# near/near-light-client

Measured on AMD Instinct MI355X. Metric: Sync/Verify proofs/sec at 1/2/4/8 MI355X + achieved HBM GB/s vs roofline, higher is better.
Workload: dtype u64 (Goldilocks field, integer)

## Files before the change

### near-light-client_amd/airgen.py

```python
import os
import sys
import types

import numpy as np

HERE = os.path.dirname(os.path.abspath(__file__))
OUT_DIR = os.path.join(HERE, "csrc", "airgen")
P = 0xFFFFFFFF00000001
MASK64 = (1 << 64) - 1

(LOCAL, NEXT, PUBLIC, CONST, ADD, SUB, MUL, EMIT_TRANSITION, EMIT_FIRST, EMIT_LAST, EMIT, PERIODIC, PACK_LOCAL, PACK_NEXT, EMIT_BOOL,
 LOADV, XOR3, CH, MAJ, SEGMENT, EMIT_LOGUP, MAC) = range(22)


def program_hash(words):
    h = 0xcbf29ce484222325
    for b in np.ascontiguousarray(words, dtype="<u8").tobytes():
        h = ((h ^ b) * 0x100000001b3) & MASK64
    return h


def canonical_words(words):
    out, i = [int(w) for w in words], 0
    while i < len(out):
        if (out[i] & 0xFF) == CONST:
            out[i + 1] %= P
            i += 2
        else:
            i += 1
    return np.array(out, dtype=np.uint64)


def _segments(words):
    segs, lo, i = [], 0, 0
    while i < len(words):
        op = int(words[i]) & 0xFF
        if op == SEGMENT:
            segs.append((lo, i))
            lo = i + 1
        i += 2 if op == CONST else 1
    segs.append((lo, len(words)))
    return segs


HORNER = "acc0 = gl::add_loose(gl::mul_loose(acc0, g.a0), %s); acc1 = gl::add_loose(gl::mul_loose(acc1, g.a1), %s);"
HORNER_SEGMENTS = {
    "ed25519_2p7_tagged": (2646, 6297, 6956, 7679, 8370, 9093, 14490, 15181, 15872),
    "sha512_tagged": (8982, 10259, 11536, 12813, 14090, 15367, 16644, 17921, 19198, 20475, 21752, 23029, 24306, 25583, 26144, 26705,
                      27266),
}


def segment_exponents(words, lo, hi):
    n, i = 0, lo
    while i < hi:
        w = int(words[i])
        op = w & 0xFF
        if op in (EMIT_TRANSITION, EMIT_FIRST, EMIT_LAST, EMIT):
            n += 1
        elif op == EMIT_LOGUP:
            n += 2
        elif op == EMIT_BOOL:
            n += ((w >> 40) & 0xFFFF) or 1
        i += 2 if op == CONST else 1
    return [n - 1 - k for k in range(n)]


class _Fold:

    def __init__(self, exponents, wide):
        self.exponents, self.wide, self.k = exponents, wide, 0

    def emit(self, lines, expr, indent="    ", canonical=False):
        if self.wide:
            e = self.exponents[self.k]
            lines.append("%sacc.mac(%s, AP0(%d), AP1(%d));" % (indent, expr if canonical else expr.replace("gl::mul(", "gl::mul_loose(", 1), e, e))
        else:
            lines.append("%sc = %s; " % (indent, expr) + HORNER % ("c", "c"))
        self.k += 1


SCHED_EVERY = 4


def _segment_body(words, lo, hi, wide=False):
    L, i, since = [], lo, 0
    fold = _Fold(segment_exponents(words, lo, hi), wide)
    R = lambda k: "r%d" % k
    while i < hi:
        if since >= SCHED_EVERY:
            L.append("    __builtin_amdgcn_sched_barrier(0);")
            since = 0
        if (int(words[i]) & 0xFF) in (LOCAL, NEXT, PUBLIC, CONST, ADD, SUB, MUL, PERIODIC, PACK_LOCAL, PACK_NEXT, XOR3, CH, MAJ, MAC):
            since += 1
        w = int(words[i])
        op, dst, a, b, sh = w & 0xFF, (w >> 8) & 0xFFFF, (w >> 24) & 0xFFFF, (w >> 40) & 0xFFFF, (w >> 56) & 0x3F
        i += 1
        if op == LOCAL:
            L.append("    %s = COL(%d, g.row);" % (R(dst), a))
        elif op == NEXT:
            L.append("    %s = COL(%d, g.row_next);" % (R(dst), a))
        elif op == PUBLIC:
            L.append("    %s = PIS(%d);" % (R(dst), a))
        elif op == PERIODIC:
            L.append("    %s = g.per[(size_t)%d * g.per_stride + g.per_off];" % (R(dst), a))
        elif op == CONST:
            L.append("    %s = 0x%016xull;" % (R(dst), int(words[i]) % P))
            i += 1
        elif op == ADD:
            L.append("    %s = gl::add(%s, mul_pow2(%s, %d));" % (R(dst), R(a), R(b), sh) if sh else "    %s = gl::add(%s, %s);" % (R(dst), R(a), R(b)))
        elif op == SUB:
            L.append("    %s = gl::sub(%s, mul_pow2(%s, %d));" % (R(dst), R(a), R(b), sh) if sh else "    %s = gl::sub(%s, %s);" % (R(dst), R(a), R(b)))
        elif op == MUL:
            L.append("    %s = gl::mul(%s, %s);" % (R(dst), R(a), R(b)))
        elif op == MAC:
            L.append("    %s = gl::add(%s, gl::mul(%s, %s));" % (R(dst), R(sh), R(a), R(b)))
        elif op == CH:
            L.append("    %s = gl::add(%s, gl::mul(%s, gl::sub(%s, %s)));" % (R(dst), R(sh), R(a), R(b), R(sh)))
        elif op in (XOR3, MAJ):
            L.append("    { const uint64_t xy = gl::mul(%s, %s), sx = gl::sub(gl::add(%s, %s), gl::add(xy, xy));" % (R(a), R(b), R(a), R(b)))
            if op == XOR3:
                L.append("      const uint64_t sz = gl::mul(sx, %s); %s = gl::sub(gl::add(sx, %s), gl::add(sz, sz)); }" % (R(sh), R(dst), R(sh)))
            else:
                L.append("      %s = gl::add(xy, gl::mul(%s, sx)); }" % (R(dst), R(sh)))
        elif op in (PACK_LOCAL, PACK_NEXT):
            row = "g.row" if op == PACK_LOCAL else "g.row_next"
            L.append("    { uint64_t v[%d];" % b)
            for k in range(b):
                L.append("      v[%d] = COL(%d, %s);" % (k, a + k, row))
            L.append("      uint64_t acc = 0;")
            for k in range(b):
                L.append("      acc = gl::add(acc, mul_pow2(v[%d], %d));" % (k, k))
            L.append("      %s = acc; }" % R(dst))
        elif op == EMIT_BOOL:
            cnt = b if b else 1
            for i0 in range(0, cnt, 8):
                m = min(8, cnt - i0)
                L.append("    { uint64_t v[%d];" % m)
                for k in range(m):
                    L.append("      v[%d] = COL(%d, g.row);" % (k, a + i0 + k))
                for k in range(m):
                    fold.emit(L, "gl::mul(v[%d], gl::sub(v[%d], 1))" % (k, k), indent="      ")
                L.append("    }")
        elif op == EMIT_LOGUP:
            L.append("    { const uint64_t al0 = PIS(g.n_pis + %d), al1 = PIS(g.n_pis + %d);" % (sh, sh + 1))
            L.append("      const uint64_t h0 = COL(%d, g.row), h1 = COL(%d, g.row), v1 = COL(%d, g.row);" % (b, b + 1, a))
            L.append("      uint64_t c0, c1;")
            if dst == 0xFFFF:
                L.append("      const uint64_t d0 = gl::add(al0, v1);")
                L.append("      c0 = gl::sub(gl::add(gl::mul(h0, d0), mul_pow2(gl::mul(h1, al1), 3)), gl::add(gl::mul(h1, al1), 1));")
                L.append("      c1 = gl::add(gl::mul(h0, al1), gl::mul(h1, d0));")
            else:
                L.append("      const uint64_t v2 = COL(%d, g.row);" % dst)
                L.append("      const uint64_t s2 = gl::add(gl::add(al0, al0), gl::add(v1, v2));")
                L.append("      const uint64_t a1sq = gl::mul(al1, al1);")
                L.append("      const uint64_t u0 = gl::add(gl::mul(gl::add(al0, v1), gl::add(al0, v2)), gl::sub(mul_pow2(a1sq, 3), a1sq));")
                L.append("      const uint64_t u1 = gl::mul(al1, s2);")
                L.append("      const uint64_t hu = gl::mul(h1, u1);")
                L.append("      c0 = gl::sub(gl::add(gl::mul(h0, u0), gl::sub(mul_pow2(hu, 3), hu)), s2);")
                L.append("      c1 = gl::sub(gl::add(gl::mul(h0, u1), gl::mul(h1, u0)), gl::add(al1, al1));")
            fold.emit(L, "c0", indent="      ", canonical=True)
            fold.emit(L, "c1", indent="      ", canonical=True)
            L.append("    }")
        elif op == LOADV:
            L.append("    __builtin_amdgcn_sched_barrier(0);")
        elif op == EMIT_TRANSITION:
            fold.emit(L, "gl::mul(%s, g.z_last)" % R(a))
        elif op == EMIT_FIRST:
            fold.emit(L, "gl::mul(%s, g.l_first)" % R(a))
        elif op == EMIT_LAST:
            fold.emit(L, "gl::mul(%s, g.l_last)" % R(a))
        elif op == EMIT:
            fold.emit(L, R(a), canonical=True)
        else:
            raise ValueError("unknown opcode %d at word %d" % (op, i - 1))
    assert fold.k == len(fold.exponents)
    return L


def _registers_of(words, lo, hi):
    regs, i = set(), lo
    while i < hi:
        w = int(words[i])
        op = w & 0xFF
        if op in (LOCAL, NEXT, PUBLIC, CONST, ADD, SUB, MUL, PERIODIC, PACK_LOCAL, PACK_NEXT, XOR3, CH, MAJ, MAC):
            regs.add((w >> 8) & 0xFFFF)
        i += 2 if op == CONST else 1
    return sorted(regs)


PART_WORDS = 10000


def generate_sources(name, words):
    words = canonical_words(words)
    h = program_hash(words)
    segs = _segments(words)
    parts, cur, cur_words = [], [], 0
    for lo, hi in segs:
        if cur and cur_words + (hi - lo) > PART_WORDS:
            parts.append(cur)
            cur, cur_words = [], 0
        cur.append((lo, hi))
        cur_words += hi - lo
    parts.append(cur)
    files = {}
    for pi, part in enumerate(parts):
        ns = "airgen_%s_p%d" % (name, pi)
        out = ["// GENERATED by near-light-client_amd/airgen.py from the program words of AIR '%s' (%d words, %d segments, hash 0x%016x):" % (name, len(words), len(segs), h),
               "// part %d of %d, segments starting at words %s." % (pi + 1, len(parts), ", ".join(str(lo) for lo, _ in part)),
               "// Do not edit: the interpreter k_air_quotient (stark.hip) runs the same words and is the parity reference.",
               '#include "../air_vm.hpp"', "", "namespace nlx {", "namespace %s {" % ns, "",
               "// what a segment needs of the point: passed BY VALUE (registers); the wave-uniform members are made scalar again inside",
               "// the function (readfirstlane), so a column's base address is a scalar load and its element ONE vector load",
               "// The column-pointer table and the public inputs are the same for every lane and constant for the launch: read through the",
               "// constant address space they are scalar loads (s_load), and a column's value is then ONE global load with the pointer in",
               "// SGPRs and the row's byte offset in a VGPR.  Through plain pointers hipcc made each a per-lane flat load with a wait",
               "// between the pointer and the value (two memory latencies per column, two more VGPRs per load in flight).",
               "// row / row_next are BYTE offsets (LDE rows * 8 < 2^32: the host selects these kernels for LDEs of <= 2^28 rows only).",
               "typedef const uint64_t __attribute__((address_space(4)))* airgen_kptr;",
               "typedef const char __attribute__((address_space(1)))* airgen_gptr;",
               "#define COL(c, off) (*(const uint64_t __attribute__((address_space(1)))*)((airgen_gptr)((airgen_kptr)g.cols)[c] + (off)))",
               "#define PIS(i) (((airgen_kptr)g.pis)[i])",
               "#define AP0(j) (((airgen_kptr)g.ap0)[j])",
               "#define AP1(j) (((airgen_kptr)g.ap1)[j])",
               "struct G {", "    uint64_t cols, pis, ap0, ap1; const uint64_t* per;",
               "    size_t per_stride, per_off; uint64_t a0, a1, z_last, l_first, l_last; uint32_t row, row_next, n_pis;", "};",
               "struct Acc { uint64_t a0, a1; };",
               "template <typename T> __device__ __forceinline__ T* uni(T* p) {",
               "    const uint64_t v = (uint64_t)p;",
               "    return (T*)(((uint64_t)(uint32_t)__builtin_amdgcn_readfirstlane((int)(v >> 32)) << 32) | (uint32_t)__builtin_amdgcn_readfirstlane((int)v));",
               "}",
               "__device__ __forceinline__ uint64_t uni(uint64_t v) {",
               "    return ((uint64_t)(uint32_t)__builtin_amdgcn_readfirstlane((int)(v >> 32)) << 32) | (uint32_t)__builtin_amdgcn_readfirstlane((int)v);",
               "}", ""]
        for lo, hi in part:
            regs = _registers_of(words, lo, hi)
            out.append("static __device__ __noinline__ Acc seg_%d(G gv) {" % lo)
            out.append("    G g = gv;")
            out.append("    g.cols = uni(gv.cols); g.pis = uni(gv.pis); g.per = uni(gv.per); g.per_stride = uni((uint64_t)gv.per_stride);")
            out.append("    g.a0 = uni(gv.a0); g.a1 = uni(gv.a1); g.n_pis = (uint32_t)__builtin_amdgcn_readfirstlane((int)gv.n_pis);")
            wide = lo not in HORNER_SEGMENTS.get(name, ())
            if wide:
                out.append("    g.ap0 = uni(gv.ap0); g.ap1 = uni(gv.ap1);")
                out.append("    GateAcc acc;")
                out.append("    acc.reset();")
            else:
                out.append("    uint64_t c, acc0 = 0, acc1 = 0;")
            if regs:
                out.append("    uint64_t %s;" % ", ".join("r%d" % r for r in regs))
            out += _segment_body(words, lo, hi, wide)
            if wide:
                out.append("    return Acc{GateAcc::fold_columns(acc.a, acc.kc), GateAcc::fold_columns(acc.a + 4, acc.kc + 4)};")
            else:
                out.append("    return Acc{acc0, acc1};")
            out.append("}")
            out.append("")
        out += [
            "// the interpreter's prologue and epilogue (csrc/stark.hip k_air_quotient), the program between them as a switch on the segment",
            "__global__ __launch_bounds__(AIRGEN_BLOCK) void kernel(AirParams p) {",
            "    const uint32_t sg = blockIdx.y;",
            "    const uint32_t first = p.n_seg > 1 ? p.seg[2 * sg] : 0u;",
            "    if (%s) return;   // another part's segment" % " && ".join("first != %du" % lo for lo, _ in part),
            "    const size_t pos = (size_t)blockIdx.x * blockDim.x + threadIdx.x;",
            "    const unsigned log_Q = p.log_n + p.qdb;",
            "    if (pos >> log_Q) return;",
            "    const size_t n = (size_t)1 << p.log_n;",
            "    const uint32_t rq = (uint32_t)(pos >> p.log_n), k = (uint32_t)(pos & (n - 1));",
            "    const uint32_t r = rq << (p.rate_bits - p.qdb);",
            "    const size_t qrow_next = ((size_t)rq << p.log_n) + ((k + 1) & (n - 1));",
            "    const uint64_t x = gl::mul(p.coset_base[rq], root_pow_(p.w_n_table, k, (uint32_t)(n >> 1)));",
            "    const uint64_t zh = gl::inv(p.zh_inv[rq]);",
            "    G g;",
            "    g.cols = (uint64_t)p.cols; g.pis = (uint64_t)p.pis; g.per = p.periodic; g.n_pis = p.n_pis;",
            "    g.row = (uint32_t)((((size_t)r << p.log_n) + k) << 3); g.row_next = (uint32_t)((((size_t)r << p.log_n) + ((k + 1) & (n - 1))) << 3);",
            "    g.per_stride = (size_t)1 << (p.qdb + p.period_bits);",
            "    g.per_off = ((size_t)rq << p.period_bits) + (k & ((1u << p.period_bits) - 1));",
            "    g.a0 = p.alphas[0]; g.a1 = p.alphas[1];",
            "    g.ap0 = (uint64_t)p.alpha_pows; g.ap1 = (uint64_t)(p.alpha_pows + p.alpha_stride);",
            "    g.z_last = gl::sub(x, p.g_inv); g.l_first = gl::mul(zh, p.l_inv[pos]); g.l_last = gl::mul(zh, p.l_inv[qrow_next]);",
            "    Acc acc{0, 0};",
            "    switch (first) {",
        ]
        for lo, _ in part:
            out.append("        case %d: acc = seg_%d(g); break;" % (lo, lo))
        out += [
            "        default: break;",
            "    }",
            "    const size_t Q = (size_t)1 << log_Q;",
            "    if (p.n_seg > 1) {",
            "        uint64_t* dst = p.part + (((size_t)sg * p.nc) << log_Q) + pos;",
            "        dst[0] = gl::mul(acc.a0, p.seg_mul[2 * sg]);",
            "        dst[Q] = gl::mul(acc.a1, p.seg_mul[2 * sg + 1]);",
            "        return;",
            "    }",
            "    const uint64_t zi = p.zh_inv[rq];",
            "    p.out[pos] = gl::mul(acc.a0, zi);",
            "    p.out[Q + pos] = gl::mul(acc.a1, zi);",
            "}",
            "",
            "}  // namespace %s" % ns,
            "void airgen_launch_%s_p%d(hipStream_t st, unsigned tiles, unsigned n_segments, const AirParams& p) {" % (name, pi),
            "    hipLaunchKernelGGL(%s::kernel, dim3(tiles, n_segments), dim3(AIRGEN_BLOCK), 0, st, p);" % ns,
            "}",
            "}  // namespace nlx", ""]
        files["air_%s_p%d.hip" % (name, pi)] = "\n".join(out)
    main = ["// GENERATED by near-light-client_amd/airgen.py: AIR '%s' (%d words, %d segments in %d parts, hash 0x%016x)." % (name, len(words), len(segs), len(parts), h),
            '#include "../air_vm.hpp"', "", "namespace nlx {"]
    main += ["void airgen_launch_%s_p%d(hipStream_t st, unsigned tiles, unsigned n_segments, const AirParams& p);" % (name, pi) for pi in range(len(parts))]
    main += ["static void airgen_launch_%s(hipStream_t st, unsigned tiles, unsigned n_segments, const AirParams& p) {" % name]
    main += ["    airgen_launch_%s_p%d(st, tiles, n_segments, p);" % (name, pi) for pi in range(len(parts))]
    main += ["}",
             "#if !defined(__HIP_DEVICE_COMPILE__)   // a host object (it holds a host function's address): not for the device pass",
             'extern const AirGenEntry airgen_entry_%s = {0x%016xull, %du, "%s", airgen_launch_%s};' % (name, h, len(words), name, name),
             "#endif",
             "}  // namespace nlx", ""]
    files["air_%s.hip" % name] = "\n".join(main)
    return files


def registry_source(names):
    out = ["// GENERATED by near-light-client_amd/airgen.py: the table nlx_stark_build searches (csrc/air_vm.hpp airgen_find).",
           '#include "../air_vm.hpp"', "", "namespace nlx {"]
    out += ["extern const AirGenEntry airgen_entry_%s;" % n for n in names]
    out += ["", "#if !defined(__HIP_DEVICE_COMPILE__)", "const AirGenEntry* airgen_find(uint64_t program_hash, uint32_t n_words) {",
            "    static const AirGenEntry* const table[] = {%s};" % ", ".join(["&airgen_entry_%s" % n for n in names] + ["nullptr"]),
            "    for (const AirGenEntry* const* e = table; *e; e++)",
            "        if ((*e)->program_hash == program_hash && (*e)->n_words == n_words) return *e;",
            "    return nullptr;", "}", "#endif", "}  // namespace nlx", ""]
    return "\n".join(out)


def _load_air_modules():
    if "nlx_amd" in sys.modules and hasattr(sys.modules["nlx_amd"], "stark"):
        return sys.modules["nlx_amd"]
    import importlib
    pkg = types.ModuleType("nlx_amd")
    pkg.__path__ = [HERE]
    sys.modules["nlx_amd"] = pkg
    lib = types.ModuleType("nlx_amd._lib")

    class NlxError(RuntimeError):
        pass
    lib.dll, lib.synth_dll, lib.ptr, lib.NlxError = None, None, (lambda a: None), NlxError
    sys.modules["nlx_amd._lib"] = lib
    for m in ("stark", "logup", "fp25519", "sha256_air", "sha512_air", "ed25519_air"):
        setattr(pkg, m, importlib.import_module("nlx_amd." + m))
    return pkg


def fixed_programs():
    pkg = _load_air_modules()
    progs = [("sha256_tagged", pkg.sha256_air.sha256_air(tagged=True).compile()),
             ("sha256", pkg.sha256_air.sha256_air(tagged=False).compile()),
             ("sha512_tagged", pkg.sha512_air.sha512_air(tagged=True).compile()),
             ("ed25519_2p7_tagged", pkg.ed25519_air.Ed25519Stark(7, tagged=True).stark.program)]
    return progs


def sources():
    progs = fixed_programs()
    files = {}
    for name, words in progs:
        files.update(generate_sources(name, words))
    files["registry.hip"] = registry_source([name for name, _ in progs])
    return files


def write_all(out_dir=OUT_DIR):
    os.makedirs(out_dir, exist_ok=True)
    files = sources()
    for stale in os.listdir(out_dir):
        if stale.endswith(".hip") and stale not in files:
            os.remove(os.path.join(out_dir, stale))
    for fn, text in files.items():
        path = os.path.join(out_dir, fn)
        if not os.path.exists(path) or open(path).read() != text:
            with open(path, "w") as f:
                f.write(text)
    return sorted(files)


if __name__ == "__main__":
    for fn in write_all():
        print(os.path.join(OUT_DIR, fn))
```

### near-light-client_amd/csrc/gl.hpp

```cpp
#pragma once
#include <stdint.h>
#include <stddef.h>
#include "nlx_field.h"

#if defined(__HIP__)
#include <hip/hip_runtime.h>
#define GL_HD __host__ __device__ __forceinline__
#define GL_H __host__ inline
#else
#define GL_HD inline
#define GL_H inline
#endif

namespace gl {

constexpr uint64_t P = 0xFFFFFFFF00000001ULL;
constexpr uint64_t EPS = 0xFFFFFFFFULL;
constexpr uint64_t GEN = NLX_GL_MULTIPLICATIVE_GROUP_GENERATOR;
constexpr uint64_t POW2_GEN = NLX_GL_POWER_OF_TWO_GENERATOR;
constexpr unsigned TWO_ADICITY = 32;
constexpr uint64_t W = 7;

GL_HD uint64_t mulhi64(uint64_t a, uint64_t b) {
#if defined(__HIP_DEVICE_COMPILE__)
    return __umul64hi(a, b);
#else
    return (uint64_t)(((unsigned __int128)a * b) >> 64);
#endif
}

#if defined(__HIP__)
__device__ __forceinline__ uint64_t canon(uint64_t a) {
    uint64_t t, c;
    asm("v_mad_u64_u32 %[t], %[c], -1, 1, %[a]" : [t] "=&v"(t), [c] "=s"(c) : [a] "v"(a));
    uint32_t r0, r1;
    asm("v_cndmask_b32_e64 %[r0], %[a0], %[t0], %[c]\n\t"
        "v_cndmask_b32_e64 %[r1], %[a1], %[t1], %[c]"
        : [r0] "=&v"(r0), [r1] "=v"(r1)
        : [a0] "v"((uint32_t)a), [a1] "v"((uint32_t)(a >> 32)), [t0] "v"((uint32_t)t), [t1] "v"((uint32_t)(t >> 32)), [c] "s"(c));
    return ((uint64_t)r1 << 32) | r0;
}
__device__ __forceinline__ uint64_t add(uint64_t a, uint64_t b) {
    uint32_t s0, s1;
    uint64_t c1, c2, t;
    asm("v_add_co_u32 %[s0], vcc, %[a0], %[b0]\n\t"
        "v_addc_co_u32 %[s1], %[c1], %[a1], %[b1], vcc"
        : [s0] "=&v"(s0), [s1] "=&v"(s1), [c1] "=s"(c1)
        : [a0] "v"((uint32_t)a), [a1] "v"((uint32_t)(a >> 32)), [b0] "v"((uint32_t)b), [b1] "v"((uint32_t)(b >> 32))
        : "vcc");
    const uint64_t s = ((uint64_t)s1 << 32) | s0;
    asm("v_mad_u64_u32 %[t], %[c], -1, 1, %[s]" : [t] "=&v"(t), [c] "=s"(c2) : [s] "v"(s));
    const uint64_t c = c1 | c2;
    uint32_t r0, r1;
    asm("v_cndmask_b32_e64 %[r0], %[s0], %[t0], %[c]\n\t"
        "v_cndmask_b32_e64 %[r1], %[s1], %[t1], %[c]"
        : [r0] "=&v"(r0), [r1] "=v"(r1)
        : [s0] "v"(s0), [s1] "v"(s1), [t0] "v"((uint32_t)t), [t1] "v"((uint32_t)(t >> 32)), [c] "s"(c));
    return ((uint64_t)r1 << 32) | r0;
}
__device__ __forceinline__ uint64_t sub(uint64_t a, uint64_t b) {
    uint32_t d0, d1, m;
    asm("v_sub_co_u32 %[d0], vcc, %[a0], %[b0]\n\t"
        "v_subb_co_u32 %[d1], vcc, %[a1], %[b1], vcc\n\t"
        "v_cndmask_b32_e64 %[m], 0, -1, vcc\n\t"
        "v_sub_co_u32 %[d0], vcc, %[d0], %[m]\n\t"
        "v_subbrev_co_u32 %[d1], vcc, 0, %[d1], vcc"
        : [d0] "=&v"(d0), [d1] "=&v"(d1), [m] "=&v"(m)
        : [a0] "v"((uint32_t)a), [a1] "v"((uint32_t)(a >> 32)), [b0] "v"((uint32_t)b), [b1] "v"((uint32_t)(b >> 32))
        : "vcc");
    return ((uint64_t)d1 << 32) | d0;
}
#endif
GL_H uint64_t canon(uint64_t a) { return a >= P ? a - P : a; }

GL_H uint64_t add(uint64_t a, uint64_t b) {
    uint64_t s = a + b;
    return (s < a || s >= P) ? s - P : s;
}
GL_H uint64_t sub(uint64_t a, uint64_t b) {
    uint64_t d = a - b;
    return a < b ? d + P : d;
}
GL_HD uint64_t neg(uint64_t a) { return a ? P - a : 0; }

#if defined(__HIP__)
__device__ __forceinline__ uint64_t add_loose(uint64_t a, uint64_t c) {
    uint32_t s0, s1, m;
    asm("v_add_co_u32 %[s0], vcc, %[a0], %[c0]\n\t"
        "v_addc_co_u32 %[s1], vcc, %[a1], %[c1], vcc\n\t"
        "v_cndmask_b32_e64 %[m], 0, -1, vcc"
        : [s0] "=&v"(s0), [s1] "=&v"(s1), [m] "=v"(m)
        : [a0] "v"((uint32_t)a), [a1] "v"((uint32_t)(a >> 32)), [c0] "v"((uint32_t)c), [c1] "v"((uint32_t)(c >> 32))
        : "vcc");
    uint64_t r;
    asm("v_mad_u64_u32 %[r], vcc, %[m], 1, %[s]" : [r] "=&v"(r) : [m] "v"(m), [s] "v"(((uint64_t)s1 << 32) | s0) : "vcc");
    return r;
}
#endif
GL_H uint64_t add_loose(uint64_t a, uint64_t c) {
    uint64_t s = a + c;
    return s < a ? s + EPS : s;
}

GL_HD uint64_t reduce128_loose(uint64_t lo, uint64_t hi) {
    uint64_t hi_hi = hi >> 32, hi_lo = hi & EPS;
    uint64_t t0 = lo - hi_hi;
    if (lo < hi_hi) t0 -= EPS;
    uint64_t t1 = (hi_lo << 32) - hi_lo;
    uint64_t r = t0 + t1;
    if (r < t1) r += EPS;
    return r;
}
GL_HD uint64_t reduce128(uint64_t lo, uint64_t hi) { return canon(reduce128_loose(lo, hi)); }

#if defined(__HIP_DEVICE_COMPILE__)
__device__ __forceinline__ uint64_t mul_loose_asm(uint64_t a, uint64_t b) {
    const uint32_t a0 = (uint32_t)a, a1 = (uint32_t)(a >> 32), b0 = (uint32_t)b, b1 = (uint32_t)(b >> 32);
    const uint64_t p0 = (uint64_t)a0 * b0;
    const uint64_t p1 = (uint64_t)a0 * b1 + (p0 >> 32);
    const uint64_t p2 = (uint64_t)a1 * b0 + (uint32_t)p1;
    uint64_t p3 = (uint64_t)a1 * b1 + (p1 >> 32), sink;
    asm("v_mad_u64_u32 %0, %1, %2, 1, %3" : "=v"(p3), "=s"(sink) : "v"((uint32_t)(p2 >> 32)), "v"(p3));
    uint32_t r0, r1, t0;
    const uint32_t w2 = (uint32_t)p3;
    asm("v_sub_co_u32 %[r0], vcc, %[w0], %[w3]\n\t"
        "v_subbrev_co_u32 %[r1], vcc, 0, %[w1], vcc\n\t"
        "v_cndmask_b32_e64 %[t0], 0, -1, vcc\n\t"
        "v_sub_co_u32 %[r0], vcc, %[r0], %[t0]\n\t"
        "v_subbrev_co_u32 %[r1], vcc, 0, %[r1], vcc"
        : [r0] "=&v"(r0), [r1] "=&v"(r1), [t0] "=&v"(t0)
        : [w0] "v"((uint32_t)p0), [w1] "v"((uint32_t)p2), [w3] "v"((uint32_t)(p3 >> 32))
        : "vcc");
    const uint64_t base = ((uint64_t)r1 << 32) | r0;
    uint64_t r;
    uint32_t tm;
    asm("v_mad_u64_u32 %[r], vcc, %[w2], -1, %[base]\n\t"
        "v_cndmask_b32_e64 %[t], 0, -1, vcc\n\t"
        "v_mad_u64_u32 %[r], vcc, %[t], 1, %[r]"
        : [r] "=&v"(r), [t] "=&v"(tm)
        : [w2] "v"(w2), [base] "v"(base)
        : "vcc");
    return r;
}
#endif

#if defined(__HIP__)
template <bool CANON>
__device__ __forceinline__ uint64_t reduce160_impl(uint32_t w0, uint32_t w1, uint32_t w2, uint32_t w3, uint32_t w4) {
    uint32_t r0, r1, t0;
    asm("v_sub_co_u32 %[r0], vcc, %[w0], %[w3]\n\t"
        "v_subbrev_co_u32 %[r1], vcc, 0, %[w1], vcc\n\t"
        "v_cndmask_b32_e64 %[t0], 0, -1, vcc\n\t"
        "v_sub_co_u32 %[r0], vcc, %[r0], %[t0]\n\t"
        "v_subbrev_co_u32 %[r1], vcc, 0, %[r1], vcc"
        : [r0] "=&v"(r0), [r1] "=&v"(r1), [t0] "=&v"(t0)
        : [w0] "v"(w0), [w1] "v"(w1), [w3] "v"(w3)
        : "vcc");
    const uint64_t base = ((uint64_t)r1 << 32) | r0;
    uint64_t r;
    uint32_t tm;
    asm("v_mad_u64_u32 %[r], vcc, %[w2], -1, %[base]\n\t"
        "v_cndmask_b32_e64 %[t], 0, -1, vcc\n\t"
        "v_mad_u64_u32 %[r], vcc, %[t], 1, %[r]"
        : [r] "=&v"(r), [t] "=&v"(tm)
        : [w2] "v"(w2), [base] "v"(base)
        : "vcc");
    return sub(CANON ? canon(r) : r, (uint64_t)w4 << 32);
}
__device__ __forceinline__ uint64_t reduce160(uint32_t w0, uint32_t w1, uint32_t w2, uint32_t w3, uint32_t w4) {
    return reduce160_impl<true>(w0, w1, w2, w3, w4);
}
__device__ __forceinline__ uint64_t reduce160_loose(uint32_t w0, uint32_t w1, uint32_t w2, uint32_t w3, uint32_t w4) {
    return reduce160_impl<false>(w0, w1, w2, w3, w4);
}
struct Wide128 {
    uint32_t w0, w1;
    uint64_t w32;
};
__device__ __forceinline__ Wide128 mul_wide(uint64_t a, uint64_t b) {
    const uint32_t a0 = (uint32_t)a, a1 = (uint32_t)(a >> 32), b0 = (uint32_t)b, b1 = (uint32_t)(b >> 32);
    const uint64_t p0 = (uint64_t)a0 * b0;
    const uint64_t p1 = (uint64_t)a0 * b1 + (p0 >> 32);
    const uint64_t p2 = (uint64_t)a1 * b0 + (uint32_t)p1;
    uint64_t p3 = (uint64_t)a1 * b1 + (p1 >> 32), sink;
    asm("v_mad_u64_u32 %0, %1, %2, 1, %3" : "=v"(p3), "=s"(sink) : "v"((uint32_t)(p2 >> 32)), "v"(p3));
    return Wide128{(uint32_t)p0, (uint32_t)p2, p3};
}
#endif

GL_HD uint64_t mul_loose(uint64_t a, uint64_t b) {
#if defined(__HIP_DEVICE_COMPILE__)
    return mul_loose_asm(a, b);
#else
    return reduce128_loose(a * b, mulhi64(a, b));
#endif
}
GL_HD uint64_t mul(uint64_t a, uint64_t b) { return canon(mul_loose(a, b)); }
GL_HD uint64_t sqr(uint64_t a) { return mul(a, a); }

GL_HD uint64_t pow(uint64_t b, uint64_t e) {
    uint64_t r = 1;
    while (e) {
        if (e & 1) r = mul(r, b);
        b = sqr(b);
        e >>= 1;
    }
    return r;
}
GL_HD uint64_t exp_pow2(uint64_t a, unsigned k) {
    while (k--) a = sqr(a);
    return a;
}
GL_HD uint64_t inv(uint64_t a) {
    uint64_t t2 = mul(sqr(a), a);
    uint64_t t3 = mul(sqr(t2), a);
    uint64_t t6 = mul(exp_pow2(t3, 3), t3);
    uint64_t t12 = mul(exp_pow2(t6, 6), t6);
    uint64_t t24 = mul(exp_pow2(t12, 12), t12);
    uint64_t t30 = mul(exp_pow2(t24, 6), t6);
    uint64_t t31 = mul(sqr(t30), a);
    uint64_t t32 = mul(sqr(t31), a);
    return mul(exp_pow2(t31, 33), t32);
}
GL_HD uint64_t root_of_unity(unsigned n_log) { return exp_pow2(POW2_GEN, TWO_ADICITY - n_log); }

struct Ext {
    uint64_t a, b;
};
GL_HD Ext ext(uint64_t a, uint64_t b = 0) { return Ext{a, b}; }
GL_HD Ext add(Ext x, Ext y) { return Ext{add(x.a, y.a), add(x.b, y.b)}; }
GL_HD Ext sub(Ext x, Ext y) { return Ext{sub(x.a, y.a), sub(x.b, y.b)}; }
#if defined(__HIP__)
template <bool CANON>
__device__ __forceinline__ Ext mul_impl(Ext x, Ext y) {
    const Wide128 ab = mul_wide(x.a, y.b), ba = mul_wide(x.b, y.a);
    uint32_t s0, s1, s2, s3, s4;
    asm("v_add_co_u32 %[s0], vcc, %[x0], %[y0]\n\t"
        "v_addc_co_u32 %[s1], vcc, %[x1], %[y1], vcc\n\t"
        "v_addc_co_u32 %[s2], vcc, %[x2], %[y2], vcc\n\t"
        "v_addc_co_u32 %[s3], vcc, %[x3], %[y3], vcc\n\t"
        "v_addc_co_u32 %[s4], vcc, 0, 0, vcc"
        : [s0] "=&v"(s0), [s1] "=&v"(s1), [s2] "=&v"(s2), [s3] "=&v"(s3), [s4] "=&v"(s4)
        : [x0] "v"(ab.w0), [x1] "v"(ab.w1), [x2] "v"((uint32_t)ab.w32), [x3] "v"((uint32_t)(ab.w32 >> 32)), [y0] "v"(ba.w0),
          [y1] "v"(ba.w1), [y2] "v"((uint32_t)ba.w32), [y3] "v"((uint32_t)(ba.w32 >> 32))
        : "vcc");
    const uint64_t c1 = reduce160_impl<CANON>(s0, s1, s2, s3, s4);
    __builtin_amdgcn_sched_barrier(0);
    const Wide128 aa = mul_wide(x.a, y.a), bb = mul_wide(x.b, y.b);
    const uint64_t t0 = (uint64_t)bb.w0 * (uint32_t)W + aa.w0;
    const uint64_t t1 = (uint64_t)bb.w1 * (uint32_t)W + (((uint64_t)aa.w1) + (t0 >> 32));
    const uint64_t t2 = (uint64_t)(uint32_t)bb.w32 * (uint32_t)W + ((aa.w32 & EPS) + (t1 >> 32));
    const uint64_t t3 = (uint64_t)(uint32_t)(bb.w32 >> 32) * (uint32_t)W + ((aa.w32 >> 32) + (t2 >> 32));
    const uint64_t c0 = reduce160_impl<CANON>((uint32_t)t0, (uint32_t)t1, (uint32_t)t2, (uint32_t)t3, (uint32_t)(t3 >> 32));
    return Ext{c0, c1};
}
__device__ __forceinline__ Ext mul(Ext x, Ext y) { return mul_impl<true>(x, y); }
__device__ __forceinline__ Ext mul_loose(Ext x, Ext y) { return mul_impl<false>(x, y); }
#endif
GL_H Ext mul(Ext x, Ext y) {
    uint64_t bb = mul(x.b, y.b);
    uint64_t c0 = add(mul(x.a, y.a), reduce128(bb * W, mulhi64(bb, W)));
    uint64_t c1 = add(mul(x.a, y.b), mul(x.b, y.a));
    return Ext{c0, c1};
}
GL_HD Ext mul(Ext x, uint64_t s) { return Ext{mul(x.a, s), mul(x.b, s)}; }
GL_HD Ext inv(Ext x) {
    uint64_t n = sub(sqr(x.a), mul(W, sqr(x.b)));
    uint64_t ni = inv(n);
    return Ext{mul(x.a, ni), mul(neg(x.b), ni)};
}
GL_HD Ext pow(Ext b, uint64_t e) {
    Ext r{1, 0};
    while (e) {
        if (e & 1) r = mul(r, b);
        b = mul(b, b);
        e >>= 1;
    }
    return r;
}
GL_HD bool eq(Ext x, Ext y) { return x.a == y.a && x.b == y.b; }

GL_HD uint32_t bitrev32(uint32_t x, unsigned bits) {
#if defined(__HIP_DEVICE_COMPILE__)
    return bits ? (__brev(x) >> (32 - bits)) : 0;
#else
    uint32_t r = 0;
    for (unsigned i = 0; i < bits; i++) r |= ((x >> i) & 1u) << (bits - 1 - i);
    return r;
#endif
}

}
```

### near-light-client_amd/csrc/gl32.hpp

```cpp
#pragma once
#include "gl.hpp"
#include "poseidon_blocks.inc"

namespace gl32 {

struct F {
    uint32_t lo, hi;
};

__device__ __forceinline__ F from_u64(uint64_t x) { return F{(uint32_t)x, (uint32_t)(x >> 32)}; }
__device__ __forceinline__ uint64_t to_u64(F x) { return ((uint64_t)x.hi << 32) | x.lo; }

__device__ __forceinline__ F add_w2_eps(uint64_t base, uint32_t w2) {
    uint64_t r;
    uint32_t t;
    asm("v_mad_u64_u32 %[r], vcc, %[w2], -1, %[base]\n\t"
        "v_cndmask_b32_e64 %[t], 0, -1, vcc\n\t"
        "v_mad_u64_u32 %[r], vcc, %[t], 1, %[r]"
        : [r] "=&v"(r), [t] "=&v"(t)
        : [w2] "v"(w2), [base] "v"(base)
        : "vcc");
    return from_u64(r);
}

__device__ __forceinline__ F reduce128(uint32_t w0, uint32_t w1, uint32_t w2, uint32_t w3) {
    uint32_t r0, r1, t0;
    asm("v_sub_co_u32 %[r0], vcc, %[w0], %[w3]\n\t"
        "v_subbrev_co_u32 %[r1], vcc, 0, %[w1], vcc\n\t"
        "v_cndmask_b32_e64 %[t0], 0, -1, vcc\n\t"
        "v_sub_co_u32 %[r0], vcc, %[r0], %[t0]\n\t"
        "v_subbrev_co_u32 %[r1], vcc, 0, %[r1], vcc"
        : [r0] "=&v"(r0), [r1] "=&v"(r1), [t0] "=&v"(t0)
        : [w0] "v"(w0), [w1] "v"(w1), [w3] "v"(w3)
        : "vcc");
    return add_w2_eps(((uint64_t)r1 << 32) | r0, w2);
}

__device__ __forceinline__ uint64_t mad_u64_one(uint32_t a, uint64_t c);

__device__ __forceinline__ F mul(F a, F b) {
#ifdef NLX_GL32_MUL_CARRY_CHAINS
    uint64_t t = (uint64_t)a.lo * b.lo;
    uint64_t m = (uint64_t)a.lo * b.hi;
    uint64_t x = (uint64_t)a.hi * b.hi;
    uint64_t mid;
    uint32_t x1;
    asm("v_mad_u64_u32 %[mid], vcc, %[ah], %[bl], %[m]\n\t"
        "v_addc_co_u32 %[x1], vcc, 0, %[xh], vcc"
        : [mid] "=&v"(mid), [x1] "=v"(x1)
        : [ah] "v"(a.hi), [bl] "v"(b.lo), [m] "v"(m), [xh] "v"((uint32_t)(x >> 32))
        : "vcc");
    uint32_t r0, r1, w1, w2, w3, t0;
    asm("v_add_co_u32 %[w1], vcc, %[th], %[m0]\n\t"
        "v_addc_co_u32 %[w2], vcc, %[x0], %[m1], vcc\n\t"
        "v_addc_co_u32 %[w3], vcc, 0, %[x1], vcc\n\t"
        "v_sub_co_u32 %[r0], vcc, %[w0], %[w3]\n\t"
        "v_subbrev_co_u32 %[r1], vcc, 0, %[w1], vcc\n\t"
        "v_cndmask_b32_e64 %[t0], 0, -1, vcc\n\t"
        "v_sub_co_u32 %[r0], vcc, %[r0], %[t0]\n\t"
        "v_subbrev_co_u32 %[r1], vcc, 0, %[r1], vcc"
        : [r0] "=&v"(r0), [r1] "=&v"(r1), [w1] "=&v"(w1), [w2] "=&v"(w2), [w3] "=&v"(w3), [t0] "=&v"(t0)
        : [w0] "v"((uint32_t)t), [th] "v"((uint32_t)(t >> 32)), [m0] "v"((uint32_t)mid), [x0] "v"((uint32_t)x),
          [m1] "v"((uint32_t)(mid >> 32)), [x1] "v"(x1)
        : "vcc");
    return add_w2_eps(((uint64_t)r1 << 32) | r0, w2);
#else
    const uint64_t p0 = (uint64_t)a.lo * b.lo;
    const uint64_t p1 = (uint64_t)a.lo * b.hi + (p0 >> 32);
    const uint64_t p2 = (uint64_t)a.hi * b.lo + (uint32_t)p1;
    uint64_t p3 = (uint64_t)a.hi * b.hi + (p1 >> 32);
    p3 = mad_u64_one((uint32_t)(p2 >> 32), p3);
    return reduce128((uint32_t)p0, (uint32_t)p2, (uint32_t)p3, (uint32_t)(p3 >> 32));
#endif
}

__device__ __forceinline__ F add_const(F a, uint64_t c) {
    F r;
    uint32_t t;
    asm("v_add_co_u32 %[r0], vcc, %[a0], %[c0]\n\t"
        "v_addc_co_u32 %[r1], vcc, %[a1], %[c1], vcc\n\t"
        "v_cndmask_b32_e64 %[t], 0, -1, vcc\n\t"
        "v_add_co_u32 %[r0], vcc, %[r0], %[t]\n\t"
        "v_addc_co_u32 %[r1], vcc, 0, %[r1], vcc"
        : [r0] "=&v"(r.lo), [r1] "=&v"(r.hi), [t] "=&v"(t)
        : [a0] "v"(a.lo), [a1] "v"(a.hi), [c0] "s"((uint32_t)c), [c1] "v"((uint32_t)(c >> 32))
        : "vcc");
    return r;
}

__device__ __forceinline__ F add_const_v(F a, uint64_t c) {
    F r;
    uint32_t t;
    asm("v_add_co_u32 %[r0], vcc, %[a0], %[c0]\n\t"
        "v_addc_co_u32 %[r1], vcc, %[a1], %[c1], vcc\n\t"
        "v_cndmask_b32_e64 %[t], 0, -1, vcc\n\t"
        "v_add_co_u32 %[r0], vcc, %[r0], %[t]\n\t"
        "v_addc_co_u32 %[r1], vcc, 0, %[r1], vcc"
        : [r0] "=&v"(r.lo), [r1] "=&v"(r.hi), [t] "=&v"(t)
        : [a0] "v"(a.lo), [a1] "v"(a.hi), [c0] "v"((uint32_t)c), [c1] "v"((uint32_t)(c >> 32))
        : "vcc");
    return r;
}

__device__ __forceinline__ F sbox7(F x) {
    F x2 = mul(x, x);
    F x4 = mul(x2, x2);
    F x3 = mul(x, x2);
    return mul(x3, x4);
}

__device__ __forceinline__ F fold_acc(uint64_t al, uint64_t ah) {
    uint64_t t;
    asm("v_mad_u64_u32 %[t], vcc, %[ah1], -1, %[al]" : [t] "=&v"(t) : [ah1] "v"((uint32_t)(ah >> 32)), [al] "v"(al) : "vcc");
    uint32_t r1, m;
    asm("v_add_co_u32 %[r1], vcc, %[t1], %[ah0]\n\t"
        "v_cndmask_b32_e64 %[m], 0, -1, vcc"
        : [r1] "=v"(r1), [m] "=v"(m)
        : [t1] "v"((uint32_t)(t >> 32)), [ah0] "v"((uint32_t)ah)
        : "vcc");
    uint64_t r;
    asm("v_mad_u64_u32 %[r], vcc, %[m], 1, %[base]" : [r] "=&v"(r) : [m] "v"(m), [base] "v"(((uint64_t)r1 << 32) | (uint32_t)t) : "vcc");
    return from_u64(r);
}

__device__ __forceinline__ void mds_layer(F (&s)[12], const uint64_t* __restrict__ rc_next = nullptr) {
    constexpr uint32_t C[12] = {17, 15, 41, 16, 2, 28, 13, 13, 39, 18, 34, 20};
    F o[12];
#pragma unroll
    for (int r = 0; r < 12; r++) {
        uint64_t al = 0, ah = 0;
        if (rc_next) {
            const uint64_t c = rc_next[r];
            al = (uint32_t)c;
            ah = c >> 32;
        }
#pragma unroll
        for (int i = 0; i < 12; i++) {
            al += (uint64_t)s[(i + r) % 12].lo * C[i];
            ah += (uint64_t)s[(i + r) % 12].hi * C[i];
        }
        if (r == 0) {
            al += (uint64_t)s[0].lo * 8u;
            ah += (uint64_t)s[0].hi * 8u;
        }
        o[r] = fold_acc(al, ah);
    }
#pragma unroll
    for (int i = 0; i < 12; i++) s[i] = o[i];
}


typedef int i32x4_t __attribute__((ext_vector_type(4)));
typedef int i32x16_t __attribute__((ext_vector_type(16)));

__device__ __forceinline__ void keep_whole(const i32x16_t& d) { asm volatile("" : : "v"(d)); }

__device__ __forceinline__ i32x4_t mds_a_fragment(uint32_t lane = threadIdx.x & 63) {
    constexpr int C[12] = {17, 15, 41, 16, 2, 28, 13, 13, 39, 18, 34, 20};
    const uint32_t rho = lane & 31, h = lane >> 5;
    const uint32_t g = (rho >> 2) & 1, r = (rho & 3) + 4 * (rho >> 3);
    uint32_t w[4] = {0, 0, 0, 0};
    if (h == g && rho < 24) {
#pragma unroll
        for (int j = 0; j < 12; j++) {
            uint32_t m = 0;
#pragma unroll
            for (int rr = 0; rr < 12; rr++)
                if ((uint32_t)rr == r) m = (uint32_t)C[(j - rr + 12) % 12] + ((rr == 0 && j == 0) ? 8u : 0u);
            w[j >> 2] |= m << (8 * (j & 3));
        }
        w[3] = r == 0 ? 0x00F88080u : 0x00008080u;
    }
    i32x4_t a;
    a.x = (int)w[0]; a.y = (int)w[1]; a.z = (int)w[2]; a.w = (int)w[3];
    return a;
}
constexpr uint32_t MDS_B_BIAS_SLOTS = 0x00808080u;

__device__ __forceinline__ void transpose_bytes4(uint32_t x0, uint32_t x1, uint32_t x2, uint32_t x3, uint32_t (&p)[4]) {
    const uint32_t t01l = __builtin_amdgcn_perm(x1, x0, 0x05010400u), t01h = __builtin_amdgcn_perm(x1, x0, 0x07030602u);
    const uint32_t t23l = __builtin_amdgcn_perm(x3, x2, 0x05010400u), t23h = __builtin_amdgcn_perm(x3, x2, 0x07030602u);
    p[0] = __builtin_amdgcn_perm(t23l, t01l, 0x05040100u);
    p[1] = __builtin_amdgcn_perm(t23l, t01l, 0x07060302u);
    p[2] = __builtin_amdgcn_perm(t23h, t01h, 0x05040100u);
    p[3] = __builtin_amdgcn_perm(t23h, t01h, 0x07060302u);
}
__device__ __forceinline__ uint64_t mad_u64(uint32_t a, uint32_t b, uint64_t c) {
    uint64_t r, sink;
    asm("v_mad_u64_u32 %0, %1, %2, %3, %4" : "=v"(r), "=s"(sink) : "v"(a), "v"(b), "v"(c));
    return r;
}
__device__ __forceinline__ uint64_t mad_u64_sc(uint32_t a, uint32_t b, uint64_t c_uniform) {
    uint64_t r, sink;
    asm("v_mad_u64_u32 %0, %1, %2, %3, %4" : "=v"(r), "=s"(sink) : "v"(a), "v"(b), "s"(c_uniform));
    return r;
}
__device__ __forceinline__ uint64_t mad_u64_one(uint32_t a, uint64_t c) {
    uint64_t r, sink;
    asm("v_mad_u64_u32 %0, %1, %2, 1, %3" : "=v"(r), "=s"(sink) : "v"(a), "v"(c));
    return r;
}
__device__ __forceinline__ F fold_pair(uint64_t t, uint32_t yh, uint32_t k16) {
    uint64_t z, u, sink, sink2;
    asm("v_mad_u64_u32 %0, %1, %2, %3, 0" : "=v"(z), "=s"(sink) : "v"(yh), "v"(k16));
    asm("v_mad_u64_u32 %0, %1, %2, -1, %3" : "=v"(u), "=s"(sink2) : "v"((uint32_t)(z >> 32)), "v"(t));
    uint32_t r1, m;
    asm("v_add_co_u32 %0, vcc, %2, %3\n\t"
        "v_cndmask_b32_e64 %1, 0, -1, vcc"
        : "=v"(r1), "=v"(m)
        : "v"((uint32_t)(u >> 32)), "v"((uint32_t)z)
        : "vcc");
    return from_u64(mad_u64_one(m, ((uint64_t)r1 << 32) | (uint32_t)u));
}

template <int RC>
__device__ __forceinline__ void mds_layer_mfma(F (&s)[12], const i32x4_t a, const uint64_t* __restrict__ rcb) {
    uint32_t k16 = 65536u, bw = MDS_B_BIAS_SLOTS;
    asm("" : "+v"(k16));
    asm("" : "+v"(bw));
    i32x16_t zero;
#pragma unroll
    for (int i = 0; i < 16; i++) zero[i] = 0;
    uint32_t x[2][12], y[2][12];
#pragma unroll
    for (int half = 0; half < 2; half++) {
// ... 178 lines not shown
```

Before: 23.43.

## Restructure Goldilocks multiply carry chain and reduction, add three-wave launch bounds

Rewrites the 64x64 Goldilocks multiply so the carry from the middle partial product is kept in an SGPR pair and folded into the reduction's first subtract. This removes the separate mad-by-one carry-propagation instruction. An optional shorter reduction variant is added behind a macro, and the shared core now backs gl32 and the extension-field multiply. Separately, selected generated AIR kernel parts for sha512_tagged get a min-waves-per-EU launch bound of 3, which caps register use to raise occupancy but risks spills.

```diff
diff --git a/near-light-client_amd/airgen.py b/near-light-client_amd/airgen.py
--- a/near-light-client_amd/airgen.py
+++ b/near-light-client_amd/airgen.py
@@ -79,6 +79,8 @@
             lines.append("%sc = %s; " % (indent, expr) + HORNER % ("c", "c"))
         self.k += 1
 
+
+THREE_WAVE_PARTS = {"sha512_tagged": (1, 2)}
 
 SCHED_EVERY = 4
 
@@ -258,7 +260,7 @@
             out.append("")
         out += [
             "// the interpreter's prologue and epilogue (csrc/stark.hip k_air_quotient), the program between them as a switch on the segment",
-            "__global__ __launch_bounds__(AIRGEN_BLOCK) void kernel(AirParams p) {",
+            "__global__ __launch_bounds__(AIRGEN_BLOCK%s) void kernel(AirParams p) {" % (", 3" if pi in THREE_WAVE_PARTS.get(name, ()) else ""),
             "    const uint32_t sg = blockIdx.y;",
             "    const uint32_t first = p.n_seg > 1 ? p.seg[2 * sg] : 0u;",
             "    if (%s) return;   // another part's segment" % " && ".join("first != %du" % lo for lo, _ in part),
diff --git a/near-light-client_amd/csrc/gl.hpp b/near-light-client_amd/csrc/gl.hpp
--- a/near-light-client_amd/csrc/gl.hpp
+++ b/near-light-client_amd/csrc/gl.hpp
@@ -113,24 +113,64 @@
 }
 GL_HD uint64_t reduce128(uint64_t lo, uint64_t hi) { return canon(reduce128_loose(lo, hi)); }
 
-#if defined(__HIP_DEVICE_COMPILE__)
-__device__ __forceinline__ uint64_t mul_loose_asm(uint64_t a, uint64_t b) {
-    const uint32_t a0 = (uint32_t)a, a1 = (uint32_t)(a >> 32), b0 = (uint32_t)b, b1 = (uint32_t)(b >> 32);
+#if defined(__HIP__)
+#if defined(NLX_FIELD_MUL_PARENT)
+constexpr bool MUL_HAS_K = false;
+#else
+constexpr bool MUL_HAS_K = true;
+#endif
+struct Wide128 {
+    uint32_t w0, w1;
+    uint64_t w32;
+    uint64_t k;
+};
+__device__ __forceinline__ Wide128 mul_chain(uint32_t a0, uint32_t a1, uint32_t b0, uint32_t b1) {
     const uint64_t p0 = (uint64_t)a0 * b0;
     const uint64_t p1 = (uint64_t)a0 * b1 + (p0 >> 32);
+#if defined(NLX_FIELD_MUL_PARENT)
     const uint64_t p2 = (uint64_t)a1 * b0 + (uint32_t)p1;
     uint64_t p3 = (uint64_t)a1 * b1 + (p1 >> 32), sink;
     asm("v_mad_u64_u32 %0, %1, %2, 1, %3" : "=v"(p3), "=s"(sink) : "v"((uint32_t)(p2 >> 32)), "v"(p3));
+    return Wide128{(uint32_t)p0, (uint32_t)p2, p3, 0};
+#else
+    uint64_t p2, k;
+    asm("v_mad_u64_u32 %0, %1, %2, %3, %4" : "=v"(p2), "=&s"(k) : "v"(a1), "v"(b0), "v"(p1));
+    const uint64_t p3 = (uint64_t)a1 * b1 + (p2 >> 32);
+    return Wide128{(uint32_t)p0, (uint32_t)p2, p3, k};
+#endif
+}
+__device__ __forceinline__ Wide128 fold_k(Wide128 x) {
+#if !defined(NLX_FIELD_MUL_PARENT)
+    uint32_t w3;
+    uint64_t sink;
+    asm("v_addc_co_u32_e64 %0, %1, 0, %2, %3" : "=v"(w3), "=&s"(sink) : "v"((uint32_t)(x.w32 >> 32)), "s"(x.k));
+    x.w32 = ((uint64_t)w3 << 32) | (uint32_t)x.w32;
+#endif
+    return x;
+}
+
+#define NLX_GL_SUB_W3_K "v_subb_co_u32_e64 %[r0], vcc, %[w0], %[w3], %[k]\n\t"
+#define NLX_GL_SUB_W3 "v_sub_co_u32 %[r0], vcc, %[w0], %[w3]\n\t"
+template <bool HAS_K>
+__device__ __forceinline__ uint64_t reduce128_core(uint32_t w0, uint32_t w1, uint32_t w2, uint32_t w3, uint64_t k) {
+#if !defined(NLX_FIELD_REDUCE7)
+#define NLX_GL_REPAIR                                \
+    "v_subbrev_co_u32 %[r1], vcc, 0, %[w1], vcc\n\t" \
+    "v_cndmask_b32_e64 %[t0], 0, -1, vcc\n\t"        \
+    "v_sub_co_u32 %[r0], vcc, %[r0], %[t0]\n\t"      \
+    "v_subbrev_co_u32 %[r1], vcc, 0, %[r1], vcc"
     uint32_t r0, r1, t0;
-    const uint32_t w2 = (uint32_t)p3;
-    asm("v_sub_co_u32 %[r0], vcc, %[w0], %[w3]\n\t"
-        "v_subbrev_co_u32 %[r1], vcc, 0, %[w1], vcc\n\t"
-        "v_cndmask_b32_e64 %[t0], 0, -1, vcc\n\t"
-        "v_sub_co_u32 %[r0], vcc, %[r0], %[t0]\n\t"
-        "v_subbrev_co_u32 %[r1], vcc, 0, %[r1], vcc"
-        : [r0] "=&v"(r0), [r1] "=&v"(r1), [t0] "=&v"(t0)
-        : [w0] "v"((uint32_t)p0), [w1] "v"((uint32_t)p2), [w3] "v"((uint32_t)(p3 >> 32))
-        : "vcc");
+    if constexpr (HAS_K)
+        asm(NLX_GL_SUB_W3_K NLX_GL_REPAIR
+            : [r0] "=&v"(r0), [r1] "=&v"(r1), [t0] "=&v"(t0)
+            : [w0] "v"(w0), [w1] "v"(w1), [w3] "v"(w3), [k] "s"(k)
+            : "vcc");
+    else
+        asm(NLX_GL_SUB_W3 NLX_GL_REPAIR
+            : [r0] "=&v"(r0), [r1] "=&v"(r1), [t0] "=&v"(t0)
+            : [w0] "v"(w0), [w1] "v"(w1), [w3] "v"(w3)
+            : "vcc");
+#undef NLX_GL_REPAIR
     const uint64_t base = ((uint64_t)r1 << 32) | r0;
     uint64_t r;
     uint32_t tm;
@@ -141,30 +181,50 @@
         : [w2] "v"(w2), [base] "v"(base)
         : "vcc");
     return r;
-}
-#endif
-
-#if defined(__HIP__)
-template <bool CANON>
-__device__ __forceinline__ uint64_t reduce160_impl(uint32_t w0, uint32_t w1, uint32_t w2, uint32_t w3, uint32_t w4) {
-    uint32_t r0, r1, t0;
-    asm("v_sub_co_u32 %[r0], vcc, %[w0], %[w3]\n\t"
-        "v_subbrev_co_u32 %[r1], vcc, 0, %[w1], vcc\n\t"
-        "v_cndmask_b32_e64 %[t0], 0, -1, vcc\n\t"
-        "v_sub_co_u32 %[r0], vcc, %[r0], %[t0]\n\t"
-        "v_subbrev_co_u32 %[r1], vcc, 0, %[r1], vcc"
-        : [r0] "=&v"(r0), [r1] "=&v"(r1), [t0] "=&v"(t0)
-        : [w0] "v"(w0), [w1] "v"(w1), [w3] "v"(w3)
-        : "vcc");
+#else
+#define NLX_GL_REPAIR                                \
+    "v_subbrev_co_u32 %[r1], vcc, 0, %[w1], vcc\n\t" \
+    "v_subbrev_co_u32_e64 %[m], %[bad], 0, %[w2], vcc"
+    uint32_t r0, r1, m;
+    uint64_t bad;
+    if constexpr (HAS_K)
+        asm(NLX_GL_SUB_W3_K NLX_GL_REPAIR
+            : [r0] "=&v"(r0), [r1] "=&v"(r1), [m] "=&v"(m), [bad] "=&s"(bad)
+            : [w0] "v"(w0), [w1] "v"(w1), [w2] "v"(w2), [w3] "v"(w3), [k] "s"(k)
+            : "vcc");
+    else
+        asm(NLX_GL_SUB_W3 NLX_GL_REPAIR
+            : [r0] "=&v"(r0), [r1] "=&v"(r1), [m] "=&v"(m), [bad] "=&s"(bad)
+            : [w0] "v"(w0), [w1] "v"(w1), [w2] "v"(w2), [w3] "v"(w3)
+            : "vcc");
+#undef NLX_GL_REPAIR
     const uint64_t base = ((uint64_t)r1 << 32) | r0;
-    uint64_t r;
-    uint32_t tm;
-    asm("v_mad_u64_u32 %[r], vcc, %[w2], -1, %[base]\n\t"
-        "v_cndmask_b32_e64 %[t], 0, -1, vcc\n\t"
-        "v_mad_u64_u32 %[r], vcc, %[t], 1, %[r]"
-        : [r] "=&v"(r), [t] "=&v"(tm)
-        : [w2] "v"(w2), [base] "v"(base)
-        : "vcc");
+    uint64_t u;
+    uint32_t t, lo, hi;
+    asm("v_mad_u64_u32 %[u], vcc, %[m], -1, %[base]\n\t"
+        "v_cndmask_b32_e64 %[t], 0, -1, vcc"
+        : [u] "=&v"(u), [t] "=&v"(t)
+        : [m] "v"(m), [base] "v"(base)
+        : "vcc");
+    asm("v_addc_co_u32_e64 %[lo], vcc, %[u0], %[t], %[bad]\n\t"
+        "v_addc_co_u32 %[hi], vcc, 0, %[u1], vcc"
+        : [lo] "=&v"(lo), [hi] "=v"(hi)
+        : [u0] "v"((uint32_t)u), [u1] "v"((uint32_t)(u >> 32)), [t] "v"(t), [bad] "s"(bad)
+        : "vcc");
+    return ((uint64_t)hi << 32) | lo;
+#endif
+}
+#undef NLX_GL_SUB_W3_K
+#undef NLX_GL_SUB_W3
+
+__device__ __forceinline__ uint64_t mul_loose_asm(uint64_t a, uint64_t b) {
+    const Wide128 x = mul_chain((uint32_t)a, (uint32_t)(a >> 32), (uint32_t)b, (uint32_t)(b >> 32));
+    return reduce128_core<MUL_HAS_K>(x.w0, x.w1, (uint32_t)x.w32, (uint32_t)(x.w32 >> 32), x.k);
+}
+
+template <bool CANON, bool HAS_K = false>
+__device__ __forceinline__ uint64_t reduce160_impl(uint32_t w0, uint32_t w1, uint32_t w2, uint32_t w3, uint32_t w4, uint64_t k = 0) {
+    const uint64_t r = reduce128_core<HAS_K>(w0, w1, w2, w3, k);
     return sub(CANON ? canon(r) : r, (uint64_t)w4 << 32);
 }
 __device__ __forceinline__ uint64_t reduce160(uint32_t w0, uint32_t w1, uint32_t w2, uint32_t w3, uint32_t w4) {
@@ -173,18 +233,8 @@
 __device__ __forceinline__ uint64_t reduce160_loose(uint32_t w0, uint32_t w1, uint32_t w2, uint32_t w3, uint32_t w4) {
     return reduce160_impl<false>(w0, w1, w2, w3, w4);
 }
-struct Wide128 {
-    uint32_t w0, w1;
-    uint64_t w32;
-};
 __device__ __forceinline__ Wide128 mul_wide(uint64_t a, uint64_t b) {
-    const uint32_t a0 = (uint32_t)a, a1 = (uint32_t)(a >> 32), b0 = (uint32_t)b, b1 = (uint32_t)(b >> 32);
-    const uint64_t p0 = (uint64_t)a0 * b0;
-    const uint64_t p1 = (uint64_t)a0 * b1 + (p0 >> 32);
-    const uint64_t p2 = (uint64_t)a1 * b0 + (uint32_t)p1;
-    uint64_t p3 = (uint64_t)a1 * b1 + (p1 >> 32), sink;
-    asm("v_mad_u64_u32 %0, %1, %2, 1, %3" : "=v"(p3), "=s"(sink) : "v"((uint32_t)(p2 >> 32)), "v"(p3));
-    return Wide128{(uint32_t)p0, (uint32_t)p2, p3};
+    return mul_chain((uint32_t)a, (uint32_t)(a >> 32), (uint32_t)b, (uint32_t)(b >> 32));
 }
 #endif
 
@@ -233,7 +283,7 @@
 #if defined(__HIP__)
 template <bool CANON>
 __device__ __forceinline__ Ext mul_impl(Ext x, Ext y) {
-    const Wide128 ab = mul_wide(x.a, y.b), ba = mul_wide(x.b, y.a);
+    const Wide128 ab = mul_wide(x.a, y.b), ba = fold_k(mul_wide(x.b, y.a));
     uint32_t s0, s1, s2, s3, s4;
     asm("v_add_co_u32 %[s0], vcc, %[x0], %[y0]\n\t"
         "v_addc_co_u32 %[s1], vcc, %[x1], %[y1], vcc\n\t"
@@ -244,14 +294,14 @@
         : [x0] "v"(ab.w0), [x1] "v"(ab.w1), [x2] "v"((uint32_t)ab.w32), [x3] "v"((uint32_t)(ab.w32 >> 32)), [y0] "v"(ba.w0),
           [y1] "v"(ba.w1), [y2] "v"((uint32_t)ba.w32), [y3] "v"((uint32_t)(ba.w32 >> 32))
         : "vcc");
-    const uint64_t c1 = reduce160_impl<CANON>(s0, s1, s2, s3, s4);
+    const uint64_t c1 = reduce160_impl<CANON, MUL_HAS_K>(s0, s1, s2, s3, s4, ab.k);
     __builtin_amdgcn_sched_barrier(0);
-    const Wide128 aa = mul_wide(x.a, y.a), bb = mul_wide(x.b, y.b);
+    const Wide128 aa = mul_wide(x.a, y.a), bb = fold_k(mul_wide(x.b, y.b));
     const uint64_t t0 = (uint64_t)bb.w0 * (uint32_t)W + aa.w0;
     const uint64_t t1 = (uint64_t)bb.w1 * (uint32_t)W + (((uint64_t)aa.w1) + (t0 >> 32));
     const uint64_t t2 = (uint64_t)(uint32_t)bb.w32 * (uint32_t)W + ((aa.w32 & EPS) + (t1 >> 32));
     const uint64_t t3 = (uint64_t)(uint32_t)(bb.w32 >> 32) * (uint32_t)W + ((aa.w32 >> 32) + (t2 >> 32));
-    const uint64_t c0 = reduce160_impl<CANON>((uint32_t)t0, (uint32_t)t1, (uint32_t)t2, (uint32_t)t3, (uint32_t)(t3 >> 32));
+    const uint64_t c0 = reduce160_impl<CANON, MUL_HAS_K>((uint32_t)t0, (uint32_t)t1, (uint32_t)t2, (uint32_t)t3, (uint32_t)(t3 >> 32), aa.k);
     return Ext{c0, c1};
 }
 __device__ __forceinline__ Ext mul(Ext x, Ext y) { return mul_impl<true>(x, y); }
diff --git a/near-light-client_amd/csrc/gl32.hpp b/near-light-client_amd/csrc/gl32.hpp
--- a/near-light-client_amd/csrc/gl32.hpp
+++ b/near-light-client_amd/csrc/gl32.hpp
@@ -24,16 +24,7 @@
 }
 
 __device__ __forceinline__ F reduce128(uint32_t w0, uint32_t w1, uint32_t w2, uint32_t w3) {
-    uint32_t r0, r1, t0;
-    asm("v_sub_co_u32 %[r0], vcc, %[w0], %[w3]\n\t"
-        "v_subbrev_co_u32 %[r1], vcc, 0, %[w1], vcc\n\t"
-        "v_cndmask_b32_e64 %[t0], 0, -1, vcc\n\t"
-        "v_sub_co_u32 %[r0], vcc, %[r0], %[t0]\n\t"
-        "v_subbrev_co_u32 %[r1], vcc, 0, %[r1], vcc"
-        : [r0] "=&v"(r0), [r1] "=&v"(r1), [t0] "=&v"(t0)
-        : [w0] "v"(w0), [w1] "v"(w1), [w3] "v"(w3)
-        : "vcc");
-    return add_w2_eps(((uint64_t)r1 << 32) | r0, w2);
+    return from_u64(gl::reduce128_core<false>(w0, w1, w2, w3, 0));
 }
 
 __device__ __forceinline__ uint64_t mad_u64_one(uint32_t a, uint64_t c);
@@ -65,12 +56,8 @@
         : "vcc");
     return add_w2_eps(((uint64_t)r1 << 32) | r0, w2);
 #else
-    const uint64_t p0 = (uint64_t)a.lo * b.lo;
-    const uint64_t p1 = (uint64_t)a.lo * b.hi + (p0 >> 32);
-    const uint64_t p2 = (uint64_t)a.hi * b.lo + (uint32_t)p1;
-    uint64_t p3 = (uint64_t)a.hi * b.hi + (p1 >> 32);
-    p3 = mad_u64_one((uint32_t)(p2 >> 32), p3);
-    return reduce128((uint32_t)p0, (uint32_t)p2, (uint32_t)p3, (uint32_t)(p3 >> 32));
+    const gl::Wide128 x = gl::mul_chain(a.lo, a.hi, b.lo, b.hi);
+    return from_u64(gl::reduce128_core<gl::MUL_HAS_K>(x.w0, x.w1, (uint32_t)x.w32, (uint32_t)(x.w32 >> 32), x.k));
 #endif
 }
 
```

Measured after the change: 24.37, median of 6. 1.04x the previous value.
